# imjaegyun/super_resolution

Hardware: AMD Instinct MI355X
Metric: SR output megapixels/sec, HAT-S x4, 1280x720 LR in (higher is better)
Workload: dtype bf16; 1 GPU; HAT-S x4, one 3x720x1280 LR frame per GPU, full-frame forward; upscale=4, parallelism=dp1

## Files before the change

include/hat_mi355x.h:

```cpp
#ifndef HAT_MI355X_H
#define HAT_MI355X_H

#include <stdint.h>

#ifdef __cplusplus
extern "C" {
#endif

#define HAT_ABI_VERSION 2

enum { HAT_F32 = 0, HAT_BF16 = 1 };
enum { HAT_EINVAL = -1, HAT_ELDS = -2, HAT_EUNSUPPORTED = -3 };

enum { HAT_ACT_NONE = 0, HAT_ACT_GELU = 1 , HAT_ACT_LRELU = 2 ,
       HAT_ACT_LRELU02 = 3  };
enum { HAT_X_NHWC_T = 0, HAT_X_NHWC_F32 = 1, HAT_X_NCHW_F32_MEAN = 2 };
enum { HAT_O_NHWC_T = 0, HAT_O_NHWC_F32 = 1, HAT_O_PIXSHUF_T = 2, HAT_O_NCHW_F32 = 3,
       HAT_O_FOLD2_NCHW_F32 = 4  };

typedef struct HatConvDesc {
    const void* x;
    const void* x0;
    const void* w;
    const float* bias;
// ... 38 lines not shown
int hat_conv3x3_small(const HatConvDesc* d, void* stream);

typedef struct HatCabFoldDesc {
    const void* c1;
    const float* c1_colsum;
    const float* w2;
    const float* b2;
    const float* wk;
    const float* bias_in;
    float* scale;
    void* wf;
    float* bias_out;
    float* tmp;
    int32_t B, H, W, C, mid, ld1, tiles, ldcs, k, ld_scale, dtype;
    float conv_scale;
    const float* stats;
    const float* w2f;
} HatCabFoldDesc;
int hat_cab_fold(const HatCabFoldDesc* d, void* stream);

typedef struct HatAggrCabDesc {
    HatConvDesc lin;
    const void* c1;
    const void* wf;
    const float* bias_b;
} HatAggrCabDesc;
int hat_aggr_cab(const HatAggrCabDesc* d, void* stream);

int hat_layernorm_blocks(void);
int hat_layernorm(const float* x, void* y, const float* gamma, const float* beta, float* gap_partial,
                  int32_t B, int64_t npix, int32_t C, int32_t ldy, int32_t out_f32, int32_t gap_c,
                  int32_t dtype, void* stream);

int hat_add_f32(const float* a, const float* c, float* out, int32_t B, int64_t n, int64_t c_bstride, void* stream);

int hat_esc_weights(const float* gap_partial, int32_t nblk, int64_t npix, const float* w1, const float* b1,
                    const float* w2, const float* b2, const float* plk_packed, void* w_out, int32_t B,
                    int32_t pdim, int32_t ksize, int32_t Kpad, int32_t dtype, void* stream);

int hat_esc_conv13(const void* x, int32_t ldx, const void* wp, int32_t Kpad, void* y16, int32_t B, int32_t H, int32_t W,
                   int32_t dtype, void* stream);

int hat_eca_scale(const float* colsum, int32_t tiles, int32_t ldc, int64_t npix, const float* wk, int32_t k,
                  float conv_scale, float* tmp, float* scale, int32_t B, int32_t C, void* stream);

int hat_dwconv_gate(const void* u, const float* wdw, const float* bdw, void* out, int32_t B, int32_t H,
                    int32_t W, int32_t hid, int32_t ldu, int32_t ldo, int32_t dtype, void* stream);

typedef struct HatMlpDesc {
    const void* x;
    const void* w1f;
    const float* b1;
    const void* w2f;
    const float* b2;
    const float* r1;
    void* out;
    int32_t B, H, W, C, hidden;
    int32_t ldx, ldr1, ldo;
    int32_t out_f32, dtype;
} HatMlpDesc;
int hat_ocab_mlp(const HatMlpDesc* d, void* stream);
int hat_ocab_qkv(const HatMlpDesc* d, void* stream);

int hat_ocab_keybias(const void* sal, int32_t ldsal, const void* kv, int32_t ldkv, float* kb, int32_t B, int32_t H, int32_t W,
                     int32_t C, int32_t ws, int32_t wse, int32_t pad, int32_t k_keep, int32_t dtype, void* stream);
int hat_ocab_attention_kb(const void* q, const void* kv, const float* bias_rot, const float* kb, void* out, int32_t B, int32_t H,
// ... 345 lines not shown
```

super_resolution_amd/_lib.py:

```python
from __future__ import annotations

import ctypes as C
import os
import threading

_HERE = os.path.dirname(os.path.abspath(__file__))
LIB_PATH = os.environ.get("HAT_MI355X_LIB") or os.path.join(_HERE, "libhat_mi355x.so")

ABI_VERSION = 2
HAT_F32, HAT_BF16 = 0, 1
ACT_NONE, ACT_GELU, ACT_LRELU, ACT_LRELU02 = 0, 1, 2, 3
X_NHWC_T, X_NHWC_F32, X_NCHW_F32_MEAN = 0, 1, 2
O_NHWC_T, O_NHWC_F32, O_PIXSHUF_T, O_NCHW_F32, O_FOLD2_NCHW_F32 = 0, 1, 2, 3, 4
METRICS_Y, METRICS_BGR, METRICS_PSNR, METRICS_SSIM = 1, 2, 4, 8

_ERRORS = {-1: "HAT_EINVAL (bad argument)", -2: "HAT_ELDS (tile does not fit in 160 KiB LDS)",
           -3: "HAT_EUNSUPPORTED (shape not instantiated)"}


class HatConvDesc(C.Structure):
    _fields_ = [
        ("x", C.c_void_p), ("x0", C.c_void_p), ("w", C.c_void_p), ("bias", C.c_void_p),
        ("out", C.c_void_p), ("r1", C.c_void_p), ("r2", C.c_void_p), ("r2scale", C.c_void_p), ("colsum", C.c_void_p),
        ("B", C.c_int32), ("H", C.c_int32), ("W", C.c_int32),
# ... 71 lines not shown
class HatNafHalfDesc(C.Structure):
    _fields_ = [("r_in", C.c_void_p), ("gprev", C.c_void_p), ("wf", C.c_void_p), ("bf", C.c_void_p), ("r_out", C.c_void_p),
                ("w1", C.c_void_p), ("b1", C.c_void_p), ("dww", C.c_void_p), ("dwb", C.c_void_p), ("g_out", C.c_void_p),
                ("partials", C.c_void_p), ("wf_bstride", C.c_int64), ("bf_bstride", C.c_int32),
                ("B", C.c_int32), ("H", C.c_int32), ("W", C.c_int32), ("C", C.c_int32), ("ldr", C.c_int32), ("ldg", C.c_int32),
                ("ldo", C.c_int32), ("dtype", C.c_int32), ("reserved0", C.c_int32)]


class HatNafFoldDesc(C.Structure):
    _fields_ = [("partials", C.c_void_p), ("wsca", C.c_void_p), ("bsca", C.c_void_p), ("w2", C.c_void_p), ("b2", C.c_void_p),
                ("beta", C.c_void_p), ("wf", C.c_void_p), ("bf", C.c_void_p), ("npix", C.c_int64),
                ("B", C.c_int32), ("tiles", C.c_int32), ("C", C.c_int32), ("dtype", C.c_int32)]


class HatEscConvFfnDesc(C.Structure):
    _fields_ = [("x", C.c_void_p), ("ln_g", C.c_void_p), ("ln_b", C.c_void_p), ("w1", C.c_void_p), ("b1", C.c_void_p),
                ("dww", C.c_void_p), ("dwb", C.c_void_p), ("w2", C.c_void_p), ("b2", C.c_void_p), ("r", C.c_void_p),
                ("out", C.c_void_p), ("partials", C.c_void_p), ("ln_eps", C.c_float),
                ("B", C.c_int32), ("H", C.c_int32), ("W", C.c_int32), ("hid_p", C.c_int32), ("ldx", C.c_int32), ("ldr", C.c_int32),
                ("ldo", C.c_int32), ("out_f32", C.c_int32), ("dtype", C.c_int32), ("reserved0", C.c_int32)]


class HatVggConvDesc(C.Structure):
    _fields_ = [("x", C.c_void_p), ("w", C.c_void_p), ("bias", C.c_void_p), ("slope", C.c_void_p), ("out", C.c_void_p),
                ("B", C.c_int32), ("H", C.c_int32), ("W", C.c_int32), ("ldx", C.c_int32), ("ldo", C.c_int32), ("frame", C.c_int32),
                ("dtype", C.c_int32), ("reserved0", C.c_int32)]


class HatRdbConvDesc(C.Structure):
    _fields_ = [("x", C.c_void_p), ("w", C.c_void_p), ("bias", C.c_void_p), ("out", C.c_void_p), ("r1", C.c_void_p), ("r2", C.c_void_p),
                ("s_out", C.c_void_p), ("B", C.c_int32), ("H", C.c_int32), ("W", C.c_int32), ("cin", C.c_int32), ("cout", C.c_int32),
                ("ldx", C.c_int32), ("ldo", C.c_int32), ("out_off", C.c_int32), ("slope", C.c_float), ("beta1", C.c_float),
                ("beta2", C.c_float), ("dtype", C.c_int32)]


_YUV_BLOCK = [C.c_void_p, C.c_int64, C.c_int64, C.c_void_p, C.c_void_p, C.c_int64, C.c_int32, C.c_int64]

SIGNATURES = {
    "hat_abi_version": (C.c_int, []),
    "hat_target_arch": (C.c_char_p, []),
    "hat_conv_tiles": (C.c_int, [C.POINTER(HatConvDesc), C.POINTER(C.c_int32)]),
    "hat_ocab_mlp": (C.c_int, [C.POINTER(HatMlpDesc), C.c_void_p]),
    "hat_ocab_qkv": (C.c_int, [C.POINTER(HatMlpDesc), C.c_void_p]),
    "hat_conv_occupancy": (C.c_int, [C.POINTER(HatConvDesc), C.POINTER(C.c_int32)]),
    "hat_conv_plan": (C.c_int, [C.POINTER(HatConvDesc), C.POINTER(C.c_int32), C.POINTER(C.c_int32), C.POINTER(C.c_int32),
                                C.POINTER(C.c_int64)]),
    "hat_conv": (C.c_int, [C.POINTER(HatConvDesc), C.c_void_p]),
    "hat_linear": (C.c_int, [C.POINTER(HatConvDesc), C.c_void_p]),
    "hat_conv_guarded": (C.c_int, [C.POINTER(HatConvDesc), C.c_void_p, C.c_void_p]),
    "hat_linear_guarded": (C.c_int, [C.POINTER(HatConvDesc), C.c_void_p, C.c_void_p]),
    "hat_hab_tail3_guarded": (C.c_int, [C.POINTER(HatHabTailDesc), C.c_void_p, C.c_void_p]),
    "hat_conv3x3_small_groups": (C.c_int, [C.POINTER(HatConvDesc), C.POINTER(C.c_int32)]),
    "hat_conv3x3_small": (C.c_int, [C.POINTER(HatConvDesc), C.c_void_p]),
    "hat_cab_fold": (C.c_int, [C.POINTER(HatCabFoldDesc), C.c_void_p]),
    "hat_aggr_cab": (C.c_int, [C.POINTER(HatAggrCabDesc), C.c_void_p]),
    "hat_ffn_tiles": (C.c_int, [C.POINTER(HatFfnDesc), C.POINTER(C.c_int32)]),
    "hat_ffn": (C.c_int, [C.POINTER(HatFfnDesc), C.c_void_p]),
    "hat_ffn2": (C.c_int, [C.POINTER(HatFfnDesc), C.c_void_p]),
    "hat_hab_tail": (C.c_int, [C.POINTER(HatHabTailDesc), C.c_void_p]),
    "hat_hab_tail3": (C.c_int, [C.POINTER(HatHabTailDesc), C.c_void_p]),
    "hat_plan_load": (C.c_int, [C.c_char_p, C.POINTER(C.c_void_p)]),
    "hat_plan_info": (C.c_int, [C.c_void_p, C.POINTER(C.c_int32), C.POINTER(C.c_int64), C.POINTER(C.c_int64)]),
    "hat_plan_forward": (C.c_int, [C.c_void_p, C.c_void_p, C.c_void_p, C.c_void_p]),
    "hat_plan_free": (None, [C.c_void_p]),
    "hat_layernorm_blocks": (C.c_int, []),
    "hat_layernorm": (C.c_int, [C.c_void_p, C.c_void_p, C.c_void_p, C.c_void_p, C.c_void_p, C.c_int32, C.c_int64,
# ... 95 lines not shown
    "hat_niqe_block_stats": (C.c_int, [C.c_void_p, C.c_int32, C.c_int32, C.c_int32, C.c_int32, C.POINTER(C.c_double), C.c_void_p,
                                       C.c_void_p]),
    "hat_naf_half_tiles": (C.c_int, [C.c_int32, C.c_int32]),
    "hat_naf_half": (C.c_int, [C.POINTER(HatNafHalfDesc), C.c_void_p]),
    "hat_naf_fold": (C.c_int, [C.POINTER(HatNafFoldDesc), C.c_void_p]),
    "hat_esc_convffn_tiles": (C.c_int, [C.c_int32, C.c_int32]),
    "hat_esc_convffn": (C.c_int, [C.POINTER(HatEscConvFfnDesc), C.c_void_p]),
    "hat_window_attention_r": (C.c_int, [C.c_void_p] * 4 + [C.c_int32] * 10 + [C.c_void_p]),
    "hat_esc_layernorm": (C.c_int, [C.c_void_p] * 4 + [C.c_float, C.c_int64, C.c_int32, C.c_int32, C.c_int32, C.c_void_p]),
    "hat_esc_shuffle_add": (C.c_int, [C.c_void_p] * 3 + [C.c_int32] * 5 + [C.c_void_p]),
    "hat_escreal_skip": (C.c_int, [C.c_void_p] * 7 + [C.c_int32] * 6 + [C.c_void_p]),
    "hat_dysample": (C.c_int, [C.c_void_p] * 4 + [C.c_int32] * 5 + [C.c_void_p]),
    "hat_unshuffle_pad": (C.c_int, [C.c_void_p] * 2 + [C.c_int32] * 5 + [C.c_void_p]),
    "hat_escrealm_skip": (C.c_int, [C.c_void_p] * 9 + [C.c_int32] * 8 + [C.c_void_p]),
    "hat_shuffle_planes": (C.c_int, [C.c_void_p] * 2 + [C.c_int32] * 5 + [C.c_void_p]),
    "hat_escfp_convffn": (C.c_int, [C.POINTER(HatEscConvFfnDesc), C.c_void_p]),
    "hat_escfp_layernorm": (C.c_int, [C.c_void_p] * 4 + [C.c_float, C.c_int64, C.c_int32, C.c_int32, C.c_int32, C.c_void_p]),
    "hat_escfp_weights": (C.c_int, [C.c_void_p, C.c_int32, C.c_int64] + [C.c_void_p] * 7 + [C.c_int32] * 3 + [C.c_void_p]),
    "hat_escfp_shuffle_bicubic": (C.c_int, [C.c_void_p] * 4 + [C.c_int32] * 5 + [C.c_void_p]),
    "hat_lte_query": (C.c_int, [C.c_void_p, C.c_void_p, C.c_int32, C.c_int32, C.c_void_p, C.c_int32, C.c_int32] + [C.c_void_p] * 11
                      + [C.c_int64, C.c_int32, C.c_int32] + [C.c_float] * 4 + [C.c_void_p, C.c_int32, C.c_void_p]),
    "hat_lte_query_u8": (C.c_int, [C.c_void_p, C.c_void_p, C.c_int32, C.c_int32, C.c_void_p, C.c_int32, C.c_int32] + [C.c_void_p] * 9
                         + [C.c_int32, C.c_int32] + [C.c_float] * 4 + [C.c_void_p, C.c_int64, C.c_int32, C.c_int32, C.c_void_p]),
    "hat_lte_query_yuv": (C.c_int, [C.c_void_p, C.c_void_p, C.c_int32, C.c_int32, C.c_void_p, C.c_int32, C.c_int32] + [C.c_void_p] * 9
                          + [C.c_int32, C.c_int32] + [C.c_float] * 4 + [C.POINTER(HatYuvSurface), C.c_void_p, C.c_int32, C.c_void_p]),
    "hat_shuffle_to_u8": (C.c_int, [C.c_void_p, C.c_int32, C.c_void_p] + [C.c_int32] * 4 + [C.c_void_p, C.c_int64, C.c_int64] + [C.c_int32] * 3
                          + [C.c_void_p]),
    "hat_shuffle_to_yuv": (C.c_int, [C.c_void_p, C.c_int32, C.c_void_p] + [C.c_int32] * 4 + [C.POINTER(HatYuvSurface), C.c_int32, C.c_int32,
                                                                                              C.c_void_p, C.c_void_p]),
    "hat_vgg_conv": (C.c_int, [C.POINTER(HatVggConvDesc), C.c_void_p]),
    "hat_vgg_conv_tiles": (C.c_int, [C.c_int32] * 4 + [C.POINTER(C.c_int32)] * 3),
    "hat_rdb_conv": (C.c_int, [C.POINTER(HatRdbConvDesc), C.c_void_p]),
    "hat_rdb_conv_tiles": (C.c_int, [C.c_int32] * 4 + [C.POINTER(C.c_int32)] * 3),
}

_lib = None
_lock = threading.Lock()


def load():
    global _lib
    if _lib is not None:
        return _lib
    with _lock:
        if _lib is not None:
            return _lib
        if not os.path.exists(LIB_PATH):
            raise RuntimeError(
                f"{LIB_PATH} not found: the HIP kernels are not built. Run `python -m super_resolution_amd.build` "
                "(needs hipcc). There is no CPU fallback for the HAT forward pass.")
        import torch
        lib = C.CDLL(LIB_PATH)
        for name, (res, args) in SIGNATURES.items():
            fn = getattr(lib, name, None)
            if fn is None:
                raise RuntimeError(f"{LIB_PATH} does not export `{name}` (stale build?)")
            fn.restype = res
            fn.argtypes = args
        if lib.hat_abi_version() != ABI_VERSION:
            raise RuntimeError(f"ABI version mismatch: library {lib.hat_abi_version()}, binding {ABI_VERSION} (stale or overridden "
                               f"{LIB_PATH}? rebuild with `python -m super_resolution_amd.build`)")
        _lib = lib
    return _lib


def check(rc: int, what: str):
# ... 4 lines not shown
```

super_resolution_amd/build.py:

```python
from __future__ import annotations

import os
import subprocess
import sys
from concurrent.futures import ThreadPoolExecutor

HERE = os.path.dirname(os.path.abspath(__file__))
CSRC = os.path.join(HERE, "csrc")
LIB = os.path.join(HERE, "libhat_mi355x.so")
SOURCES = ["hat_conv.hip", "hat_conv64r.hip", "hat_attn.hip", "hat_misc.hip", "hat_ffn.hip", "hat_ffn2.hip", "hat_tail3.hip", "hat_tail3l.hip", "hat_pw.hip", "hat_mlp.hip", "hat_cabsq.hip", "hat_esc13.hip", "hat_upfold.hip", "hat_u8.hip", "hat_yuv.hip", "hat_packed422.hip", "hat_resize.hip", "hat_pil_resize.hip", "hat_metrics.hip", "hat_dihedral.hip", "hat_niqe.hip", "hat_naf.hip", "hat_esc.hip", "hat_escreal.hip", "hat_escrealm.hip", "hat_escfp.hip", "hat_lte.hip", "hat_esc_sink.hip", "hat_vgg.hip", "hat_rrdb.hip", "hat_plan.cpp"]
HEADERS = [os.path.join(CSRC, "hat_common.h"), os.path.join(CSRC, "hat_yuv_check.h"), os.path.join(CSRC, "hat_packed_check.h"), os.path.join(CSRC, "hat_yuv_sample.h"), os.path.join(CSRC, "hat_frame_sink.h"), os.path.join(CSRC, "hat_esc_ffn.h"), os.path.join(CSRC, "hat_gated_ffn.h"), os.path.join(CSRC, "hat_plan_parse.h"), os.path.join(os.path.dirname(HERE), "include", "hat_mi355x.h")]
FLAGS = ["-O3", "--offload-arch=gfx950", "-fPIC", "-std=c++17", "-Wall", "-Wno-unused-function"]


def _hipcc() -> str:
    for c in (os.environ.get("HIPCC"), "/opt/rocm/bin/hipcc", "hipcc"):
        if c and (os.path.isabs(c) and os.path.exists(c) or not os.path.isabs(c)):
            return c
    raise RuntimeError("hipcc not found")


def _stale(target: str, deps) -> bool:
    if not os.path.exists(target):
        return True
    t = os.path.getmtime(target)
    return any(os.path.getmtime(d) > t for d in deps)


def build(force: bool = False, verbose: bool = True) -> str:
    hipcc = _hipcc()
    objs, jobs = [], []
    for src in SOURCES:
        s = os.path.join(CSRC, src)
        o = os.path.join(CSRC, os.path.splitext(src)[0] + ".o")
        objs.append(o)
        if force or _stale(o, [s] + HEADERS):
            jobs.append([hipcc, *FLAGS, "-c", s, "-o", o])

    def run(cmd):
        if verbose:
            print(" ".join(cmd), flush=True)
        r = subprocess.run(cmd, capture_output=True, text=True)
        if r.returncode != 0:
# ... 14 lines not shown
```

super_resolution_amd/engine.py:

```python
from __future__ import annotations

import contextlib
import dataclasses
import math
import os
import warnings
from typing import Dict, Optional

import torch

from . import ops
from .engine_base import EngineBase
from .frame_boundary import FrameBoundary
from .ops import (ACT_GELU, ACT_LRELU, ACT_NONE, O_NCHW_F32, O_NHWC_F32, O_NHWC_T, O_PIXSHUF_T, X_NCHW_F32_MEAN, X_NHWC_F32, X_NHWC_T)
from .packing import _ESC

RGB_MEAN = (0.4488, 0.4371, 0.4040)


def _r8(x: int) -> int:
    return (x + 7) // 8 * 8


def _r4(x: int) -> int:
    return (x + 3) // 4 * 4


T16_GUARD_MODES = ("defer", "sync", "off")


@dataclasses.dataclass(frozen=True)
class Options:
    no_n16: bool = False
    no_t16: bool = False
    no_fused_ffn: bool = False
    ffn_v1: bool = False
    no_hab_tail: bool = False
    no_cab_fold: bool = False
    no_cab_sweep: bool = False
    no_esc13: bool = False
    esc_side: bool = False
    one_stream: bool = False
    no_attn_log2: bool = False
    no_ocab_mlp: bool = False
    no_ocab_qkv: bool = False
    no_bf16_conv_in: bool = False
    no_conv_ln: bool = False
    no_upfold: bool = False
    t16_guard: str = "defer"

    def __post_init__(self):
        if self.t16_guard not in T16_GUARD_MODES:
            raise ValueError(f"t16_guard / HAT_T16_GUARD is one of {', '.join(T16_GUARD_MODES)}, got {self.t16_guard!r}")

    @classmethod
    def from_env(cls, env=None) -> "Options":
        env = os.environ if env is None else env
        get = lambda name: env.get("HAT_" + name.upper(), "")
        any_value = ("no_cab_fold", "no_cab_sweep", "no_ocab_mlp", "no_ocab_qkv", "no_bf16_conv_in", "no_conv_ln")
        kw = {k.name: (get(k.name) != "" if k.name in any_value else get(k.name) == "1") for k in dataclasses.fields(cls) if k.type == "bool"}
        return cls(t16_guard=(get("t16_guard") or "defer"), **kw)


class _T16Guard:

    def __init__(self, dev):
        self.slot = torch.zeros(1, dtype=torch.int32, device=dev)
        self.host = torch.zeros(1, dtype=torch.int32).pin_memory()
        self.event = torch.cuda.Event()
        self.pending = 0

    def word(self) -> int:
        return int(self.host[0]) & 0xFFFFFFFF


class _Packed:

    def __getitem__(self, key):
        try:
            return getattr(self, key)
        except AttributeError:
# ... 250 lines not shown
            oc.fh2 = ops.pack_conv_weight(sd[p + ".focus_head.2.weight"], sd[p + ".focus_head.2.bias"], dt, dev)
        return oc

    def _pack_ps(self, sd, key, r):
        w = sd[key + ".weight"]
        o = w.shape[0]
        cps = o // (r * r)
        n = torch.arange(o)
        perm = (n % cps) * (r * r) + n // cps
        return ops.pack_conv_weight(w, sd[key + ".bias"], self.dtype, self.dev, out_perm=perm)

    def _resolve(self):
        layers, dt, C = self.layers, self.dtype, self.C
        escs = [hb.esc for G in layers for hb in G.habs] + [G.ocab.esc for G in layers if G.ocab.esc is not None]
        wide = any(e.npad > 16 for e in escs)
        for gi, G in enumerate(layers):
            oc = G.ocab
            for i, hb in enumerate(G.habs):
                nh = G.habs[i + 1] if i + 1 < len(G.habs) else None
                hb.next_ln = (nh.n1, nh.esc.pdim) if nh is not None else (oc.n1, oc.esc.pdim if oc.esc is not None else 0)
                if hb.fold is not None:
                    hb.tail = "fused144" if hb.tail144_ok and not wide else "aggr_cab"
                else:
                    hb.tail = "fused180" if hb.tail180_ok and hb.next_ln[1] <= 16 else "aggr"
            G.to_conv = bool(G.conv is not None and dt == ops.HAT_BF16 and _r8(C) == C and oc.mlp2.frag and not self.opt.no_bf16_conv_in)
            cv = G.conv
            if cv is not None and dt == ops.HAT_BF16 and not self.opt.no_conv_ln and cv.n_slices == 1 and cv.nout == cv.nt * 16:
                if gi + 1 < len(layers):
                    nhs = layers[gi + 1].habs
                    nxt, gap_c = (nhs[0].n1, nhs[0].esc.pdim) if nhs else (None, 0)
                else:
                    nxt, gap_c = (self.norm, 0) if self.conv_after_body is not None else (None, 0)
                G.conv_ln = (nxt, gap_c) if nxt is not None and gap_c in (0, 4, 8, 12, 16) else None
        self._plan_t16()
        self.u8_fused = self.conv_last_sweep is not None and self.conv_last_sweep[2] == 3
        hab0 = layers[0].habs[0] if layers and layers[0].habs else None
        self._hab0 = hab0
        self._yw = max([16] + [e.npad for e in escs])
        self._kpad = max([hab0.esc.kpad if hab0 else 0] + [G.ocab.esc.kpad for G in layers if G.ocab.esc is not None])

    def _plan_t16(self):
        layers = self.layers
        for G in layers:
            G.ocab16 = G.out16 = False
            for hb in G.habs:
                hb.out16 = False
        if not self.t16:
            return
        tail16 = lambda hb: hb.tail == "fused144" and hb.ffn3.C == 144
        conv16 = lambda G: bool(G.conv is not None and not G.conv.frag and G.conv.ksize > 1 and G.conv.nt == 9
                                and G.conv.n_slices == 1 and G.conv.nout == 144)
        for G in layers:
            oc = G.ocab
            G.ocab16 = bool(G.habs and tail16(G.habs[-1]) and G.to_conv and oc.mlpf is not None and oc.proj.frag
                            and oc.proj.nt == 9 and getattr(oc.proj, "ksplit", None) is None and oc.esc is None)
            for i, hb in enumerate(G.habs):
                hb.out16 = tail16(hb) and (G.ocab16 if i + 1 == len(G.habs) else tail16(G.habs[i + 1]))
        for gi, G in enumerate(layers):
            if not conv16(G) or G.conv_ln is None:
                continue
            if gi + 1 < len(layers):
                nG = layers[gi + 1]
                G.out16 = bool(nG.habs and tail16(nG.habs[0]) and conv16(nG))
            else:
                G.out16 = self.conv_after_body is not None

    def guarded_launches(self):
        if not self.t16 or self.t16_guard == "off":
            return []
        out = []
        for gi, G in enumerate(self.layers):
            out += [("tail", gi, i) for i, hb in enumerate(G.habs) if hb.out16]
            out += [("proj", gi)] if G.ocab16 else []
            out += [("conv", gi)] if G.out16 else []
        return out

    @contextlib.contextmanager
    def guard_mode(self, mode: str):
        if mode not in T16_GUARD_MODES:
            raise ValueError(f"t16_guard is one of {', '.join(T16_GUARD_MODES)}, got {mode!r}")
        with self._lock:
            old, self.t16_guard = self.t16_guard, mode
        try:
            yield self
        finally:
            with self._lock:
                self.t16_guard = old

    def _sat(self, stores16: bool):
        return self._guard.slot if stores16 and self._armed else None

    def _guard_begin(self) -> bool:
        g = self._guard
        if g is None:
            return False
        if g.pending and g.event.query():
            self._guard_look()
        self._armed = self.t16 and self.t16_guard != "off"
        if self._armed and not g.pending:
            g.slot.zero_()
        return self._armed

    def _guard_look(self):
        g = self._guard
        word, n, g.pending = g.word(), g.pending, 0
        if word and self.t16:
            self.t16_clipped_frames += n
            self._t16_fall_back(word)
            warnings.warn(f"the FP16 residual stream left the FP16 range (peaked at {self.t16_peak:.4g}, limit 65504): {n} frame"
                          f"{'s' if n != 1 else ''} already returned {'were' if n != 1 else 'was'} clipped; this engine carries "
                          f"the stream in fp32 from now on (t16_guard='sync' re-runs such a frame before it is returned)", RuntimeWarning, stacklevel=3)

    def _t16_fall_back(self, word: int):
        self.t16, self._armed = False, False
        self.t16_fallbacks += 1
        self.t16_peak = ops.read_sat(word)
        self._plan_t16()
        self._ws_cache.clear()

    def _guard_end(self, defer: bool = False) -> bool:
# ... 192 lines not shown
        self._upsample(f, y, sink)
        return y

    def _naf_stem(self, f: _Fwd, x):
        st, w, c = self.naf, f.w, self.naf.c
        kw = dict(B=f.B, H=f.H, W=f.W, C_=c, dtype=f.dt)
        s_in, s_out, g_in, g_out = w["naf_sA"], w["naf_sB"], w["naf_gA"], w["naf_gB"]
        ops.conv(st.head, x, s_in, **f.geo, ldx=0, ldo=c, x_mode=X_NCHW_F32_MEAN, out_mode=O_NHWC_F32)
        fold = None
        for blk in st.blocks:
            if fold is None:
                ops.naf_half(s_in, g_out, blk.w1, blk.b1, blk.dww, blk.dwb, partials=w["naf_part"], **kw)
            else:
                ops.naf_half(s_in, g_out, blk.w1, blk.b1, blk.dww, blk.dwb, gprev=g_in, wf=fold[0], bf=fold[1], r_out=s_out,
                             partials=w["naf_part"], **kw)
                s_in, s_out = s_out, s_in
            g_in, g_out = g_out, g_in
            ops.naf_fold(w["naf_part"], blk, w["naf_wf"], w["naf_bf"], **kw)
            ops.naf_half(s_in, g_out, blk.w1f, blk.b1f, blk.dwwf, blk.dwbf, gprev=g_in, wf=w["naf_wf"], wf_bstride=c * c,
                         bf=w["naf_bf"], bf_bstride=c, r_out=s_out, **kw)
            s_in, s_out = s_out, s_in
            g_in, g_out = g_out, g_in
            fold = (blk.wf2, blk.bf2)
        if fold is not None:
            ops.naf_half(s_in, None, None, None, None, None, gprev=g_in, wf=fold[0], bf=fold[1], r_out=s_out, **kw)
            s_in = s_out
        ops.conv(st.tail, s_in, w["x_naf"], **f.geo, ldx=c, ldo=0, x_mode=X_NHWC_F32, out_mode=O_NCHW_F32)
        ops.add_f32(w["x_naf"], x, w["x_naf"], B=f.B, n=x.shape[1] * f.N)
        return w["x_naf"]

    def _head(self, f: _Fwd, x):
        w, tA, C = f.w, f.w["tA"], self.C
        r = float(self.cfg.get("img_range", 1.0))
        ops.conv(self.conv_first, x, w["f0"], **f.geo, ldx=0, ldo=C, x_mode=X_NCHW_F32_MEAN, out_mode=O_NHWC_F32,
                 in_scale=r, mean=self._mean())
        if self.pe_norm is not None:
            f.ln(w["f0"], tA, self.pe_norm, out_f32=True)
        else:
            tA.copy_(w["f0"])
        if self.ape is not None:
            npix, off = (f.band.Hfull * f.W, f.band.e0 * f.W * C) if f.band is not None else (f.N, 0)
            if self.ape.numel() != npix * C:
                raise RuntimeError(f"absolute_pos_embed holds {self.ape.numel() // C} positions but the "
                                   f"{'frame' if f.band is not None else 'input'} has {npix} pixels (ape=True fixes the input "
                                   f"size to img_size, hat_arch.py:699-702)")
            ops.add_f32(tA, self.ape[off:off + f.N * C], tA, B=f.B, n=f.N * C, c_bstride=0)

    def _mean(self):
        return RGB_MEAN if self.cfg["in_chans"] == 3 else (0.0,) * 4

    def _hab_prologue(self, f: _Fwd, hb: _Hab):
        w, esc, bd = f.w, hb.esc, f.band
        if bd is not None and not f.have_n:
            yield ("halo", [(f.t, self._hab_halo(esc))])
        if not f.have_n:
            f.ln(f.t, w["n"], hb.n1, gap_c=esc.pdim)
            f.nblk, f.have_n16 = ops.layernorm_blocks(), False
        elif bd is not None:
            er = esc.ksize // 2 + 1
            yield ("halo", [(f.t, 1)] + ([(w["n"], 3), (w["n16"], er)] if f.have_n16 else [(w["n"], self._hab_halo(esc))]))
        gst = None
        if bd is not None:
            gst = f.gstat(esc)
            if f.have_n16:
                f.pooled(w["n16"], 16, esc.pdim, gst[0])
            else:
# ... 288 lines not shown
```

super_resolution_amd/ops.py:

```python
from __future__ import annotations

import collections
import ctypes as C
from typing import Optional

import numpy as np
import torch

from . import _lib
from ._lib import (ACT_GELU, ACT_LRELU, ACT_LRELU02, ACT_NONE, HAT_BF16, HAT_F32, O_FOLD2_NCHW_F32, O_NCHW_F32, O_NHWC_F32, O_NHWC_T, O_PIXSHUF_T,
                   X_NCHW_F32_MEAN, X_NHWC_F32, X_NHWC_T, HatAggrCabDesc, HatCabFoldDesc, HatConvDesc, HatFfnDesc, HatHabTailDesc, HatMlpDesc, HatNafFoldDesc,
                   HatNafHalfDesc, HatEscConvFfnDesc, HatVggConvDesc, HatRdbConvDesc)
from .packing import (ESC_HID_PAD, FP16_SAFE, KC, NAF_WIDTHS, TORCH_DTYPE, PackedConv, PackedEscFfn, PackedFFN, PackedMlp, PackedNafBlock, choose_nt,
                      esc_geo_ensemble, pack_esc_convffn, PackedEscRealSkip, ESCFP_HID_PAD, PackedEscFpLk, bicubic_phase_table, escfp_rank1_fold,
                      pack_escfp_convffn, pack_escfp_lk, dysample_fold, pack_escreal_skip, pack_nearest_conv,
                      LTE_HIDDEN, PackedLte, pack_lte,
                      PackedVggConv, pack_vgg_conv,
                      RDB_CIN, PackedRdbConv, pack_rdb_conv,
                      UNI_UPSAMPLERS, PackedEscRealMSkip, conv_nearest_fold, pack_conv_nearest, pack_escrealm_skip, pack_pixshuf_conv, pixshuf_perm,
                      choose_nt_linear, naf_ffn_fold, naf_frags, pack_naf_block,
                      ffn_fp16_range_bound, pack_upfold, pack_cab_squeeze, pack_cab_w2f, pack_conv_weight, pack_ffn, pack_ffn2, pack_ffn3,
                      pack_linear_weight, pack_ocab_mlp, pack_ocab_qkv, pack_pointwise)

DTYPE_CODE = {"f32": HAT_F32, "fp32": HAT_F32, "float32": HAT_F32, "bf16": HAT_BF16, "bfloat16": HAT_BF16}


def _ptr(t: Optional[torch.Tensor]) -> Optional[int]:
    if t is None:
        return None
    if not t.is_cuda:
        raise RuntimeError("HAT HIP ops need device tensors (no CPU path exists)")
    if not t.is_contiguous():
        raise RuntimeError("HAT HIP ops need contiguous tensors")
    return t.data_ptr()


def _stream() -> int:
    return torch.cuda.current_stream().cuda_stream


_prof = None


class profile:

# ... 76 lines not shown
    d.mean = _mean4(mean)
    d.dtype = dtype
    d.reserved0 = _stream16(r1, out, out_mode)
    name, flops = "conv_kernel", 0.0
    if _prof is not None:
        wv, pt, tl, lds = C.c_int32(0), C.c_int32(0), C.c_int32(0), C.c_int64(0)
        lib.hat_conv_plan(C.byref(d), C.byref(wv), C.byref(pt), C.byref(tl), C.byref(lds))
        name = f"conv_kernel<{_TNAME[dtype]}, {wv.value}, {pt.value}, {pw.nt}>"
        flops = 2.0 * B * H * W * (pw.ksize ** 2) * d.Cin * pw.nout + (2.0 * 9 * pw.nout * B * H * W if pw.w_bstride else 0.0)
    launch = (lambda: lib.hat_conv(C.byref(d), _stream())) if sat is None else (lambda: lib.hat_conv_guarded(C.byref(d), _sat_ptr(sat), _stream()))
    _timed(name, flops, lambda: _lib.check(launch(), f"hat_conv{'' if sat is None else '_guarded'}(k={pw.ksize}, Cin={d.Cin}, N={pw.nout})"),
           tag=f"k{pw.ksize} {d.Cin}->{pw.nout} {H}x{W} x{x_mode} o{out_mode}{' r1' if r1 is not None else ''}{' r2' if r2 is not None else ''}")


def conv_tiles(pw: PackedConv, H: int, W: int, dtype: int) -> int:
    lib = _lib.load()
    d = HatConvDesc()
    d.B, d.H, d.W, d.Cin, d.ksize, d.nt, d.n_slices, d.dtype = 1, H, W, pw.cin, pw.ksize, pw.nt, pw.n_slices, dtype
    n = C.c_int32(0)
    _lib.check(lib.hat_conv_tiles(C.byref(d), C.byref(n)), "hat_conv_tiles")
    return n.value


def layernorm_blocks() -> int:
    return _lib.load().hat_layernorm_blocks()


def layernorm(x: torch.Tensor, y: torch.Tensor, gamma: torch.Tensor, beta: torch.Tensor, *, B: int, npix: int, C_: int,
              ldy: int, out_f32: bool, dtype: int, gap: Optional[torch.Tensor] = None, gap_c: int = 0):
    lib = _lib.load()
    _timed("ln_kernel", 0.0, lambda: _lib.check(
        lib.hat_layernorm(_ptr(x), _ptr(y), _ptr(gamma), _ptr(beta), _ptr(gap), B, npix, C_, ldy, int(out_f32), gap_c, dtype,
                          _stream()), "hat_layernorm"))


def add_f32(a: torch.Tensor, c: torch.Tensor, out: torch.Tensor, *, B: int, n: int, c_bstride: Optional[int] = None):
    lib = _lib.load()
    cb = n if c_bstride is None else c_bstride
    _timed("add_f32_kernel", 0.0, lambda: _lib.check(lib.hat_add_f32(_ptr(a), _ptr(c), _ptr(out), B, n, cb, _stream()), "hat_add_f32"))


def rect_sum(x: torch.Tensor, out: torch.Tensor, tmp: torch.Tensor, counter: torch.Tensor, *, B: int, W: int, ld: int, C_: int, r0: int,
             r1: int, c0: int = 0, c1: Optional[int] = None, out_off: int = 0, dtype: Optional[int] = None):
    lib = _lib.load()
    dt = dtype if dtype is not None else (HAT_BF16 if x.dtype == torch.bfloat16 else HAT_F32)
    o = out.view(B, -1)
    bstride = x.numel() // B
    _timed("rect_sum_kernel", 0.0, lambda: _lib.check(
        lib.hat_rect_sum(_ptr(x), dt, ld, C_, W, r0, r1, c0, (W if c1 is None else c1), bstride, B, o.data_ptr() + 4 * out_off, o.shape[1],
                         _ptr(tmp), _ptr(counter), _stream()), "hat_rect_sum"))


def esc_weights(gap: torch.Tensor, nblk: int, npix: int, w1, b1, w2, b2, plk_packed, w_out, *, B: int, pdim: int,
                ksize: int, kpad: int, dtype: int):
    lib = _lib.load()
    _timed("esc_weights_kernel", 0.0, lambda: _lib.check(
        lib.hat_esc_weights(_ptr(gap), nblk, npix, _ptr(w1), _ptr(b1), _ptr(w2), _ptr(b2), _ptr(plk_packed), _ptr(w_out), B,
                            pdim, ksize, kpad, dtype, _stream()), "hat_esc_weights"))


def esc_conv13_supported(pdim: int, ksize: int, dtype: int) -> bool:
    return pdim == 16 and ksize == 13 and dtype == HAT_BF16


def esc_conv13(x, wp, y16, *, B: int, H: int, W: int, ldx: int, kpad: int, dtype: int):
    lib = _lib.load()
# ... 1328 lines not shown
```

super_resolution_amd/plan.py:

```python
from __future__ import annotations

import argparse
import bisect
import ctypes as C
import struct
import threading
from typing import List, Tuple

import torch

from . import _lib

FN_IDS = ["hat_conv", "hat_linear", "hat_conv3x3_small", "hat_cab_fold", "hat_aggr_cab", "hat_ffn", "hat_ffn2", "hat_hab_tail",
          "hat_layernorm", "hat_esc_weights", "hat_eca_scale", "hat_dwconv_gate", "hat_sgfn_gate", "hat_ocab_attention",
          "hat_window_attention", "hat_cab_squeeze", "hat_conv3x3_to_planes", "hat_add_f32", "hat_esc_conv13", "hat_ocab_keybias", "hat_ocab_attention_kb", "hat_ocab_mlp", "hat_ocab_qkv", "hat_hab_tail3", "hat_ocab_attention_log2", "hat_naf_half",
          "hat_naf_fold"]
ARG_INT, ARG_FLOAT, ARG_PTR, ARG_STRUCT, ARG_HOST, ARG_STREAM = range(6)
BUF_CONST, BUF_SCRATCH, BUF_INPUT, BUF_OUTPUT = range(4)
NULL_BUF = 0xFFFFFFFF
_EXPORT_LOCK = threading.Lock()


class _Recorder:

# ... 77 lines not shown
                    out += struct.pack("<IIQ", off, bi, bo)
            elif a[0] == "host":
                out += struct.pack("<IIII", ARG_HOST, 0, len(a[1]), 0) + pad8(a[1])
            elif a[0] == "stream":
                out += struct.pack("<II", ARG_STREAM, 0)
            elif a[0] == "ptr":
                out += struct.pack("<IIIIQ", ARG_PTR, 0, a[1], 0, a[2])
            elif a[0] == "float":
                out += struct.pack("<IId", ARG_FLOAT, 0, float(a[1]))
            elif a[0] == "int":
                out += struct.pack("<IIq", ARG_INT, 0, int(a[1]))
            else:
                raise ValueError(f"plan_bytes: unknown argument form {a[0]!r}")
    where["end"] = len(out)
    if offsets is not None:
        offsets.update(where)
    return bytes(out)


def record_plan(net, x_shape: Tuple[int, int, int, int]):
    eng = net.engine()
    dev = eng.dev
    if not hasattr(eng, "pe_norm"):
        raise NotImplementedError(f"a plan records HATEngine's call list: {type(net).__name__} cannot be exported yet (DESIGN.md §7)")
    if eng.pe_norm is None:
        raise NotImplementedError("patch_norm=False copies a tensor with a torch op, which a plan cannot record")
    B, Cin, H, W = x_shape
    x = torch.zeros(x_shape, dtype=torch.float32, device=dev)
    real = _lib.load()
    rec = _Recorder(real)
    with _EXPORT_LOCK:
        _lib._lib = rec
        try:
            with torch.no_grad(), eng.guard_mode("off"):
                y = eng.forward(x, one_stream=True)
            torch.cuda.synchronize(dev)
        finally:
            _lib._lib = real
    ws = eng._workspace(B, H, W)
    consts, scratch = [], []
    _tensors_of({k: v for k, v in eng.__dict__.items() if k not in ("_ws_cache", "_guard")}, set(), consts)
    _tensors_of(ws, set(), scratch)

    bufs, index = [], {}

    def add(t, kind):
        st = t.untyped_storage()
        key = st.data_ptr()
        if key in index:
            return
        index[key] = len(bufs)
        bufs.append({"kind": kind, "start": key, "nbytes": st.nbytes(), "storage": st, "tensor": t})

    add(x, BUF_INPUT)
    add(y, BUF_OUTPUT)
    for t in scratch:
        add(t, BUF_SCRATCH)
    for t in consts:
        add(t, BUF_CONST)
    starts = sorted((b["start"], i) for i, b in enumerate(bufs))
    keys = [s for s, _ in starts]

    def resolve(p):
        if not p:
            return NULL_BUF, 0
        k = bisect.bisect_right(keys, p) - 1
        if k >= 0:
# ... 167 lines not shown
```

Before: 357.3 MP/s.

## Fuse conv_first, patch-embed LayerNorm and first HAB LayerNorm into one head kernel

```diff
diff --git a/include/hat_mi355x.h b/include/hat_mi355x.h
--- a/include/hat_mi355x.h
+++ b/include/hat_mi355x.h
@@ -94,6 +94,28 @@
                   int32_t B, int64_t npix, int32_t C, int32_t ldy, int32_t out_f32, int32_t gap_c,
                   int32_t dtype, void* stream);
 
+typedef struct HatHeadDesc {
+    const float* x;
+    const void* w;
+    const float* bias;
+    const float* ln0_g;
+    const float* ln0_b;
+    const float* ln1_g;
+    const float* ln1_b;
+    float* f0;
+    float* t;
+    void* n;
+    void* n16;
+    float* gap_partial;
+    int32_t B, H, W, C;
+    int32_t Kpad;
+    int32_t ldn, gap_c, dtype;
+    float in_scale;
+    float mean[4];
+    int32_t reserved0;
+} HatHeadDesc;
+int hat_head_fused(const HatHeadDesc* d, void* stream);
+
 int hat_add_f32(const float* a, const float* c, float* out, int32_t B, int64_t n, int64_t c_bstride, void* stream);
 
 int hat_esc_weights(const float* gap_partial, int32_t nblk, int64_t npix, const float* w1, const float* b1,
diff --git a/super_resolution_amd/_lib.py b/super_resolution_amd/_lib.py
--- a/super_resolution_amd/_lib.py
+++ b/super_resolution_amd/_lib.py
@@ -127,6 +127,14 @@
                 ("s_out", C.c_void_p), ("B", C.c_int32), ("H", C.c_int32), ("W", C.c_int32), ("cin", C.c_int32), ("cout", C.c_int32),
                 ("ldx", C.c_int32), ("ldo", C.c_int32), ("out_off", C.c_int32), ("slope", C.c_float), ("beta1", C.c_float),
                 ("beta2", C.c_float), ("dtype", C.c_int32)]
+
+
+class HatHeadDesc(C.Structure):
+    _fields_ = [("x", C.c_void_p), ("w", C.c_void_p), ("bias", C.c_void_p), ("ln0_g", C.c_void_p), ("ln0_b", C.c_void_p),
+                ("ln1_g", C.c_void_p), ("ln1_b", C.c_void_p), ("f0", C.c_void_p), ("t", C.c_void_p), ("n", C.c_void_p),
+                ("n16", C.c_void_p), ("gap_partial", C.c_void_p), ("B", C.c_int32), ("H", C.c_int32), ("W", C.c_int32), ("C", C.c_int32),
+                ("Kpad", C.c_int32), ("ldn", C.c_int32), ("gap_c", C.c_int32), ("dtype", C.c_int32), ("in_scale", C.c_float),
+                ("mean", C.c_float * 4), ("reserved0", C.c_int32)]
 
 
 _YUV_BLOCK = [C.c_void_p, C.c_int64, C.c_int64, C.c_void_p, C.c_void_p, C.c_int64, C.c_int32, C.c_int64]
@@ -288,6 +296,7 @@
     "hat_vgg_conv_tiles": (C.c_int, [C.c_int32] * 4 + [C.POINTER(C.c_int32)] * 3),
     "hat_rdb_conv": (C.c_int, [C.POINTER(HatRdbConvDesc), C.c_void_p]),
     "hat_rdb_conv_tiles": (C.c_int, [C.c_int32] * 4 + [C.POINTER(C.c_int32)] * 3),
+    "hat_head_fused": (C.c_int, [C.POINTER(HatHeadDesc), C.c_void_p]),
 }
 
 _lib = None
diff --git a/super_resolution_amd/build.py b/super_resolution_amd/build.py
--- a/super_resolution_amd/build.py
+++ b/super_resolution_amd/build.py
@@ -8,7 +8,7 @@
 HERE = os.path.dirname(os.path.abspath(__file__))
 CSRC = os.path.join(HERE, "csrc")
 LIB = os.path.join(HERE, "libhat_mi355x.so")
-SOURCES = ["hat_conv.hip", "hat_conv64r.hip", "hat_attn.hip", "hat_misc.hip", "hat_ffn.hip", "hat_ffn2.hip", "hat_tail3.hip", "hat_tail3l.hip", "hat_pw.hip", "hat_mlp.hip", "hat_cabsq.hip", "hat_esc13.hip", "hat_upfold.hip", "hat_u8.hip", "hat_yuv.hip", "hat_packed422.hip", "hat_resize.hip", "hat_pil_resize.hip", "hat_metrics.hip", "hat_dihedral.hip", "hat_niqe.hip", "hat_naf.hip", "hat_esc.hip", "hat_escreal.hip", "hat_escrealm.hip", "hat_escfp.hip", "hat_lte.hip", "hat_esc_sink.hip", "hat_vgg.hip", "hat_rrdb.hip", "hat_plan.cpp"]
+SOURCES = ["hat_conv.hip", "hat_conv64r.hip", "hat_attn.hip", "hat_misc.hip", "hat_ffn.hip", "hat_ffn2.hip", "hat_tail3.hip", "hat_tail3l.hip", "hat_pw.hip", "hat_mlp.hip", "hat_cabsq.hip", "hat_esc13.hip", "hat_upfold.hip", "hat_u8.hip", "hat_yuv.hip", "hat_packed422.hip", "hat_resize.hip", "hat_pil_resize.hip", "hat_metrics.hip", "hat_dihedral.hip", "hat_niqe.hip", "hat_naf.hip", "hat_esc.hip", "hat_escreal.hip", "hat_escrealm.hip", "hat_escfp.hip", "hat_lte.hip", "hat_esc_sink.hip", "hat_vgg.hip", "hat_rrdb.hip", "hat_head.hip", "hat_plan.cpp"]
 HEADERS = [os.path.join(CSRC, "hat_common.h"), os.path.join(CSRC, "hat_yuv_check.h"), os.path.join(CSRC, "hat_packed_check.h"), os.path.join(CSRC, "hat_yuv_sample.h"), os.path.join(CSRC, "hat_frame_sink.h"), os.path.join(CSRC, "hat_esc_ffn.h"), os.path.join(CSRC, "hat_gated_ffn.h"), os.path.join(CSRC, "hat_plan_parse.h"), os.path.join(os.path.dirname(HERE), "include", "hat_mi355x.h")]
 FLAGS = ["-O3", "--offload-arch=gfx950", "-fPIC", "-std=c++17", "-Wall", "-Wno-unused-function"]
 
diff --git a/super_resolution_amd/csrc/hat_head.hip b/super_resolution_amd/csrc/hat_head.hip
--- /dev/null
+++ b/super_resolution_amd/csrc/hat_head.hip
@@ -0,0 +1,185 @@
+#include "hat_common.h"
+
+namespace {
+
+constexpr int HEAD_BLOCKS = 1024;
+constexpr int HEAD_WAVES = 4;
+constexpr int HC = 144, HNT = 9, HKS = 3;
+constexpr int HLDW = lds_row_elems(HKS * 32, 2);
+
+struct HeadTile {
+    float v[HKS][3];
+    unsigned ok;
+};
+
+__device__ __forceinline__ void head_ln(const f32x4 (&x)[HNT], f32x4 (&o)[HNT], const float* gm, const float* bt, int g, float invC) {
+#pragma clang fp contract(off)
+    float P[4];
+#pragma unroll
+    for (int m = 0; m < 4; ++m) {
+        float s = 0.f;
+        s += (x[m][0] + x[m][1]) + (x[m][2] + x[m][3]);
+        s += (x[m + 4][0] + x[m + 4][1]) + (x[m + 4][2] + x[m + 4][3]);
+        if (m == 0) s += (x[8][0] + x[8][1]) + (x[8][2] + x[8][3]);
+        else s += (0.f + 0.f) + (0.f + 0.f);
+        P[m] = s;
+    }
+    float s = (P[0] + P[2]) + (P[1] + P[3]);
+    s += __shfl_xor(s, 32);
+    s += __shfl_xor(s, 16);
+    const float mean = s * invC;
+    float Q[4];
+#pragma unroll
+    for (int m = 0; m < 4; ++m) {
+        float q = 0.f;
+#pragma unroll
+        for (int r = 0; r < 4; ++r) { const float dlt = x[m][r] - mean; const float sq = dlt * dlt; q = q + sq; }
+#pragma unroll
+        for (int r = 0; r < 4; ++r) { const float dlt = x[m + 4][r] - mean; const float sq = dlt * dlt; q = q + sq; }
+        if (m == 0) {
+#pragma unroll
+            for (int r = 0; r < 4; ++r) { const float dlt = x[8][r] - mean; const float sq = dlt * dlt; q = q + sq; }
+        }
+        Q[m] = q;
+    }
+    float q = (Q[0] + Q[2]) + (Q[1] + Q[3]);
+    q += __shfl_xor(q, 32);
+    q += __shfl_xor(q, 16);
+    const float rstd = 1.0f / sqrtf(__builtin_fmaf(q, invC, 1e-5f));
+#pragma unroll
+    for (int nt = 0; nt < HNT; ++nt) {
+        const f32x4 gv = *reinterpret_cast<const f32x4*>(gm + nt * 16 + 4 * g);
+        const f32x4 bv = *reinterpret_cast<const f32x4*>(bt + nt * 16 + 4 * g);
+#pragma unroll
+        for (int r = 0; r < 4; ++r) o[nt][r] = __builtin_fmaf((x[nt][r] - mean) * rstd, gv[r], bv[r]);
+    }
+}
+
+__global__ __launch_bounds__(HEAD_WAVES * 64) void head_fused_kernel(const HatHeadDesc d) {
+    using M = MT<bf16_t>;
+    __shared__ __attribute__((aligned(16))) bf16_t Ws[HC * HLDW];
+    __shared__ __attribute__((aligned(16))) float tab[5][HC];
+    __shared__ float red[HEAD_WAVES][16][16];
+    const int tid = threadIdx.x, lane = tid & 63, wave = tid >> 6, g = lane >> 4, c16 = lane & 15;
+    const int b = blockIdx.y, blk = blockIdx.x * HEAD_WAVES + wave;
+    const int H = d.H, W = d.W, npix = H * W;
+
+    {
+        const bf16_t* wg = reinterpret_cast<const bf16_t*>(d.w);
+        for (int i = tid; i < HC * 12; i += HEAD_WAVES * 64) {
+            const int row = i / 12, pc = i - row * 12;
+            *reinterpret_cast<u32x4*>(Ws + row * HLDW + pc * 8) = *reinterpret_cast<const u32x4*>(wg + (size_t)row * d.Kpad + pc * 8);
+        }
+        for (int i = tid; i < HC; i += HEAD_WAVES * 64) {
+            tab[0][i] = d.bias[i];
+            tab[1][i] = d.ln0_g[i];
+            tab[2][i] = d.ln0_b[i];
+            tab[3][i] = d.ln1_g[i];
+            tab[4][i] = d.ln1_b[i];
+        }
+    }
+    __syncthreads();
+
+    const float* xb = d.x + (size_t)b * 3 * npix;
+    float* f0b = d.f0 != nullptr ? d.f0 + (size_t)b * npix * HC : nullptr;
+    float* tb = d.t + (size_t)b * npix * HC;
+    bf16_t* nb = reinterpret_cast<bf16_t*>(d.n) + (size_t)b * npix * d.ldn;
+    bf16_t* n16b = d.n16 != nullptr ? reinterpret_cast<bf16_t*>(d.n16) + (size_t)b * npix * 16 : nullptr;
+    const float invC = 1.0f / (float)d.C;
+    const float mean0 = d.mean[0], mean1 = d.mean[1], mean2 = d.mean[2], in_scale = d.in_scale;
+    constexpr int STRIDE = HEAD_BLOCKS * 16;
+
+    auto fetch = [&](int p0, HeadTile& tl) {
+        const int p = min(p0 + c16, npix - 1);
+        const int y = p / W, x = p - y * W;
+        tl.ok = 0u;
+#pragma unroll
+        for (int ks = 0; ks < HKS; ++ks) {
+            const int tap = min(4 * ks + g, 8);
+            const int yy = y + tap / 3 - 1, xx = x + tap % 3 - 1;
+            if (4 * ks + g < 9 && yy >= 0 && yy < H && xx >= 0 && xx < W) tl.ok |= 1u << ks;
+            const size_t off = (size_t)min(max(yy, 0), H - 1) * W + min(max(xx, 0), W - 1);
+#pragma unroll
+            for (int ci = 0; ci < 3; ++ci) tl.v[ks][ci] = xb[(size_t)ci * npix + off];
+        }
+    };
+
+    f32x4 gsum = {0.f, 0.f, 0.f, 0.f};
+    HeadTile cur, nx1, nx2;
+    int p0 = blk * 16;
+    fetch(p0, cur);
+    fetch(p0 + STRIDE, nx1);
+    for (; p0 < npix; p0 += STRIDE) {
+        fetch(p0 + 2 * STRIDE, nx2);
+        f32x4 acc[HNT];
+#pragma unroll
+        for (int nt = 0; nt < HNT; ++nt) acc[nt] = f32x4{0.f, 0.f, 0.f, 0.f};
+#pragma unroll
+        for (int ks = 0; ks < HKS; ++ks) {
+            const bool in = (cur.ok >> ks) & 1u;
+            M::frag_t bf = M::zero();
+            bf[0] = to_T<bf16_t>(in ? (cur.v[ks][0] - mean0) * in_scale : 0.f);
+            bf[1] = to_T<bf16_t>(in ? (cur.v[ks][1] - mean1) * in_scale : 0.f);
+            bf[2] = to_T<bf16_t>(in ? (cur.v[ks][2] - mean2) * in_scale : 0.f);
+#pragma unroll
+            for (int nt = 0; nt < HNT; ++nt) acc[nt] = M::mma(M::load(Ws + (nt * 16 + c16) * HLDW + ks * 32 + 8 * g), bf, acc[nt]);
+        }
+        const int p = p0 + c16;
+        const bool valid = p < npix;
+        const size_t pc = (size_t)min(p, npix - 1);
+#pragma unroll
+        for (int nt = 0; nt < HNT; ++nt) {
+            acc[nt] = acc[nt] + *reinterpret_cast<const f32x4*>(&tab[0][nt * 16 + 4 * g]);
+            if (valid && f0b != nullptr) *reinterpret_cast<f32x4*>(f0b + pc * HC + nt * 16 + 4 * g) = acc[nt];
+        }
+        f32x4 tv[HNT];
+        head_ln(acc, tv, tab[1], tab[2], g, invC);
+#pragma unroll
+        for (int nt = 0; nt < HNT; ++nt)
+            if (valid) *reinterpret_cast<f32x4*>(tb + pc * HC + nt * 16 + 4 * g) = tv[nt];
+        f32x4 nv[HNT];
+        head_ln(tv, nv, tab[3], tab[4], g, invC);
+        bf16_t* nrow = nb + pc * d.ldn;
+#pragma unroll
+        for (int nt = 0; nt + 1 < HNT; nt += 2) store_pair_bf16_if(nrow, nt * 16, g, nv[nt], nv[nt + 1], valid);
+        if (valid) {
+            Vec4<bf16_t>::store(nrow + 128 + 4 * g, nv[8]);
+            if (n16b != nullptr) Vec4<bf16_t>::store(n16b + pc * 16 + 4 * g, nv[0]);
+            if (4 * g < d.gap_c) gsum += as_stored<bf16_t>(nv[0]);
+        }
+        cur = nx1;
+        nx1 = nx2;
+    }
+    if (d.gap_partial != nullptr) {
+#pragma unroll
+        for (int r = 0; r < 4; ++r) red[wave][c16][4 * g + r] = gsum[r];
+        __syncthreads();
+        if (lane < 16) {
+            float s = 0.f;
+#pragma unroll
+            for (int k = 0; k < 16; ++k) s += red[wave][k][lane];
+            d.gap_partial[((size_t)b * HEAD_BLOCKS + blk) * 16 + lane] = lane < d.gap_c ? s : 0.f;
+        }
+    }
+}
+
+bool aligned16(const void* p) { return (reinterpret_cast<uintptr_t>(p) & 15) == 0; }
+
+}
+
+extern "C" int hat_head_fused(const HatHeadDesc* d, void* stream) {
+    if (!d || !d->x || !d->w || !d->bias || !d->ln0_g || !d->ln0_b || !d->ln1_g || !d->ln1_b || !d->t || !d->n) return HAT_EINVAL;
+    if (d->B < 1 || d->B > 65535 || d->H < 1 || d->W < 1 || d->reserved0 != 0) return HAT_EINVAL;
+    if ((int64_t)d->H * d->W >= (int64_t)INT32_MAX - 3 * HEAD_BLOCKS * 16) return HAT_EINVAL;
+    if (d->Kpad < HKS * 32 || d->Kpad % 32 || d->ldn < HC || d->ldn % 8) return HAT_EINVAL;
+    if (d->gap_c < 0 || d->gap_c > 16 || d->gap_c % 4 || (d->gap_c > 0) != (d->gap_partial != nullptr)) return HAT_EINVAL;
+    if (d->dtype != HAT_F32 && d->dtype != HAT_BF16) return HAT_EINVAL;
+    if (d->dtype != HAT_BF16 || d->C != HC) return HAT_EUNSUPPORTED;
+    if ((reinterpret_cast<uintptr_t>(d->x) & 3) || !aligned16(d->w) || !aligned16(d->bias) || !aligned16(d->ln0_g) || !aligned16(d->ln0_b) ||
+        !aligned16(d->ln1_g) || !aligned16(d->ln1_b) || !aligned16(d->f0) || !aligned16(d->t) || !aligned16(d->n) || !aligned16(d->n16) ||
+        !aligned16(d->gap_partial))
+        return HAT_EINVAL;
+    dim3 grid(HEAD_BLOCKS / HEAD_WAVES, d->B), block(HEAD_WAVES * 64);
+    HAT_LAUNCH(head_fused_kernel, grid, block, 0, reinterpret_cast<hipStream_t>(stream), *d);
+    return hat_check_launch();
+}
diff --git a/super_resolution_amd/engine.py b/super_resolution_amd/engine.py
--- a/super_resolution_amd/engine.py
+++ b/super_resolution_amd/engine.py
@@ -47,6 +47,7 @@
     no_bf16_conv_in: bool = False
     no_conv_ln: bool = False
     no_upfold: bool = False
+    no_head_fused: bool = False
     t16_guard: str = "defer"
 
     def __post_init__(self):
@@ -363,6 +364,9 @@
                 else:
                     nxt, gap_c = (self.norm, 0) if self.conv_after_body is not None else (None, 0)
                 G.conv_ln = (nxt, gap_c) if nxt is not None and gap_c in (0, 4, 8, 12, 16) else None
+        hb0 = layers[0].habs[0] if layers and layers[0].habs else None
+        self.head_fused = bool(not self.opt.no_head_fused and hb0 is not None and hb0.tail == "fused144" and self.pe_norm is not None
+                               and self.ape is None and ops.head_fused_supported(self.conv_first, C, hb0.esc.pdim, dt))
         self._plan_t16()
         self.u8_fused = self.conv_last_sweep is not None and self.conv_last_sweep[2] == 3
         hab0 = layers[0].habs[0] if layers and layers[0].habs else None
@@ -417,6 +421,16 @@
         finally:
             with self._lock:
                 self.t16_guard = old
+
+    @contextlib.contextmanager
+    def head_route(self, fused: bool):
+        with self._lock:
+            old, self.head_fused = self.head_fused, bool(fused and self.head_fused)
+        try:
+            yield self
+        finally:
+            with self._lock:
+                self.head_fused = old
 
     def _sat(self, stores16: bool):
         return self._guard.slot if stores16 and self._armed else None
@@ -675,6 +689,12 @@
     def _head(self, f: _Fwd, x):
         w, tA, C = f.w, f.w["tA"], self.C
         r = float(self.cfg.get("img_range", 1.0))
+        if self.head_fused:
+            hb0 = self._hab0
+            ops.head_fused(self.conv_first, x, w["f0"], tA, w["n"], self.pe_norm, hb0.n1, B=f.B, H=f.H, W=f.W, ldn=f.ldc, dtype=f.dt,
+                           in_scale=r, mean=self._mean(), n16=(w["n16"] if self.use_n16 else None), gap=w["gap"], gap_c=hb0.esc.pdim)
+            f.have_n, f.have_n16, f.nblk = True, self.use_n16, ops.layernorm_blocks()
+            return
         ops.conv(self.conv_first, x, w["f0"], **f.geo, ldx=0, ldo=C, x_mode=X_NCHW_F32_MEAN, out_mode=O_NHWC_F32,
                  in_scale=r, mean=self._mean())
         if self.pe_norm is not None:
diff --git a/super_resolution_amd/ops.py b/super_resolution_amd/ops.py
--- a/super_resolution_amd/ops.py
+++ b/super_resolution_amd/ops.py
@@ -10,7 +10,7 @@
 from . import _lib
 from ._lib import (ACT_GELU, ACT_LRELU, ACT_LRELU02, ACT_NONE, HAT_BF16, HAT_F32, O_FOLD2_NCHW_F32, O_NCHW_F32, O_NHWC_F32, O_NHWC_T, O_PIXSHUF_T,
                    X_NCHW_F32_MEAN, X_NHWC_F32, X_NHWC_T, HatAggrCabDesc, HatCabFoldDesc, HatConvDesc, HatFfnDesc, HatHabTailDesc, HatMlpDesc, HatNafFoldDesc,
-                   HatNafHalfDesc, HatEscConvFfnDesc, HatVggConvDesc, HatRdbConvDesc)
+                   HatNafHalfDesc, HatEscConvFfnDesc, HatVggConvDesc, HatRdbConvDesc, HatHeadDesc)
 from .packing import (ESC_HID_PAD, FP16_SAFE, KC, NAF_WIDTHS, TORCH_DTYPE, PackedConv, PackedEscFfn, PackedFFN, PackedMlp, PackedNafBlock, choose_nt,
                       esc_geo_ensemble, pack_esc_convffn, PackedEscRealSkip, ESCFP_HID_PAD, PackedEscFpLk, bicubic_phase_table, escfp_rank1_fold,
                       pack_escfp_convffn, pack_escfp_lk, dysample_fold, pack_escreal_skip, pack_nearest_conv,
@@ -153,6 +153,26 @@
     _timed("ln_kernel", 0.0, lambda: _lib.check(
         lib.hat_layernorm(_ptr(x), _ptr(y), _ptr(gamma), _ptr(beta), _ptr(gap), B, npix, C_, ldy, int(out_f32), gap_c, dtype,
                           _stream()), "hat_layernorm"))
+
+
+def head_fused_supported(pw: PackedConv, C_: int, gap_c: int, dtype: int) -> bool:
+    return bool(dtype == HAT_BF16 and C_ == 144 and not pw.frag and pw.ksize == 3 and pw.cin == 3 and pw.nout == 144 and pw.nt == 9
+                and pw.n_slices == 1 and pw.kpad >= 96 and gap_c in (0, 4, 8, 12, 16))
+
+
+def head_fused(pw: PackedConv, x: torch.Tensor, f0: Optional[torch.Tensor], t: torch.Tensor, n: torch.Tensor, ln0, ln1, *, B: int, H: int,
+               W: int, ldn: int, dtype: int, in_scale: float = 1.0, mean=(0.0, 0.0, 0.0, 0.0), n16: Optional[torch.Tensor] = None,
+               gap: Optional[torch.Tensor] = None, gap_c: int = 0):
+    lib = _lib.load()
+    d = HatHeadDesc()
+    d.x, d.w, d.bias, d.f0, d.t, d.n, d.n16 = _ptr(x), _ptr(pw.w), _ptr(pw.bias), _ptr(f0), _ptr(t), _ptr(n), _ptr(n16)
+    d.ln0_g, d.ln0_b, d.ln1_g, d.ln1_b = _ptr(ln0[0]), _ptr(ln0[1]), _ptr(ln1[0]), _ptr(ln1[1])
+    d.gap_partial = _ptr(gap) if gap_c else None
+    d.B, d.H, d.W, d.C, d.Kpad, d.ldn, d.gap_c, d.dtype = B, H, W, pw.nout, pw.kpad, ldn, gap_c, dtype
+    d.in_scale, d.mean = in_scale, _mean4(mean)
+    px = float(B) * H * W
+    _timed("head_fused_kernel", px * (2.0 * 27 * 144 + 2 * 8.0 * 144), lambda: _lib.check(lib.hat_head_fused(C.byref(d), _stream()), "hat_head_fused"),
+           tag=f"3->144 {H}x{W} gap{gap_c}", nbytes=px * (12 + (576 if f0 is not None else 0) + 576 + 288 + (32 if n16 is not None else 0)))
 
 
 def add_f32(a: torch.Tensor, c: torch.Tensor, out: torch.Tensor, *, B: int, n: int, c_bstride: Optional[int] = None):
diff --git a/super_resolution_amd/plan.py b/super_resolution_amd/plan.py
--- a/super_resolution_amd/plan.py
+++ b/super_resolution_amd/plan.py
@@ -133,7 +133,7 @@
     with _EXPORT_LOCK:
         _lib._lib = rec
         try:
-            with torch.no_grad(), eng.guard_mode("off"):
+            with torch.no_grad(), eng.guard_mode("off"), eng.head_route(fused=False):
                 y = eng.forward(x, one_stream=True)
             torch.cuda.synchronize(dev)
         finally:
```

New measurement: 361.6 MP/s, median of 6. 1.01x the previous value.
